# sunshanlu/ORB_SLAM2_ROS2

Measured on AMD Instinct MI355X. Metric: stereo frames/sec (extract+match) KITTI-00 1241x376; HBM GB/s vs roofline, higher is better.
Workload: dtype u8; 1 GPU; Single 1241x376 KITTI-shaped stereo pair, 8-level pyramid, 2000 FAST+rBRIEF keypoints per image, searchByStereo; batched (512 pairs per step, 512 of them distinct synthetic frames).  `value` is DEVICE-RESIDENT; the checks, rooflines, host_io, sequence job, content sweep, CPU baseline and extra legs run with --full; io=device-resident, n_features=2000, levels=8

## Files before the change

### include/orbfe.h

```cpp
#ifndef ORBFE_H_
#define ORBFE_H_

#include <stddef.h>
#include <stdint.h>

#ifdef __cplusplus
extern "C" {
#endif

#define ORBFE_ABI_VERSION 4
#define ORBFE_MAX_LEVELS 16
#define ORBFE_DESC_BYTES 32

typedef enum orbfe_status {
  ORBFE_OK = 0,
  ORBFE_EBADARG = 1,
  ORBFE_EBADSIZE = 2,
  ORBFE_EDEVICE = 3,
  ORBFE_ECAPACITY = 4,
  ORBFE_ENOMEM = 5
} orbfe_status;

typedef struct orbfe_keypoint {
  float x, y;
// ... 427 lines not shown
orbfe_status orbfe_kfstore_erase(orbfe_kfstore* store, int32_t n, const uint64_t* ids);
orbfe_status orbfe_kfstore_size(orbfe_kfstore* store, int64_t* n_keyframes, int64_t* bytes_used, int64_t* bytes_reserved);
orbfe_status orbfe_kfstore_info_get(orbfe_kfstore* store, uint64_t id, orbfe_kfstore_info* out);
orbfe_status orbfe_kfstore_fetch(orbfe_kfstore* store, uint64_t id, orbfe_keypoint* kps, uint8_t* desc, double* depth, double* right_u,
                                 int32_t* cell_off, int32_t* cell_feat, uint32_t* nodes, int32_t* node_offsets, uint32_t* features);
orbfe_status orbfe_fuse_into_keyframes_stored(orbfe_ctx* ctx, orbfe_kfstore* store, uint64_t cur_id, int32_t n_cur, const orbfe_fuse_points* pts,
                                              int32_t n_kf, const uint64_t* target_ids, const orbfe_fuse_pose* poses ,
                                              const float* z , const orbfe_camera* cam, float bl, const float* scale_factors,
                                              int32_t n_levels, float th, float ratio, int32_t dist_threshold, int32_t* best_idx,
                                              int32_t* best_dist, uint8_t* visible);
orbfe_status orbfe_create_new_map_points_stored(orbfe_ctx* ctx, orbfe_kfstore* store, uint64_t cur_id, const orbfe_tri_state* cur, int32_t n_nb,
                                                const uint64_t* nb_ids, const orbfe_tri_state* nbs, const orbfe_camera* cam, const float* k_inv,
                                                float bl, const float* scale_factors, int32_t n_levels, orbfe_tri_record* records, int64_t cap,
                                                int64_t* n_records, int32_t* tail, int64_t tail_cap, int64_t* n_tail, uint8_t* consumed);

typedef enum orbfe_stage {
  ORBFE_STAGE_RESIZE = 0,
  ORBFE_STAGE_BLUR = 1,
  ORBFE_STAGE_FAST = 2,
  ORBFE_STAGE_QUADTREE = 3,
  ORBFE_STAGE_BRIEF = 4,
  ORBFE_STAGE_STEREO = 5,
  ORBFE_STAGE_MATCH = 6,
  ORBFE_STAGE_BA = 7,
  ORBFE_STAGE_COUNT = 8
} orbfe_stage;
orbfe_status orbfe_profile_enable(orbfe_ctx* ctx, int32_t on);
orbfe_status orbfe_profile_read(orbfe_ctx* ctx, double* ms , int64_t* launches , int32_t reset);
const char* orbfe_stage_name(int32_t stage);

orbfe_status orbfe_debug_candidates(orbfe_ctx* ctx, int32_t slot, int32_t level, float* xyr, int32_t cap, int32_t* n_out);
orbfe_status orbfe_debug_se3_oplus(orbfe_ctx* ctx, int32_t n, const double* poses , const double* upd ,
                                   double* out );

#ifdef __cplusplus
}
#endif
#endif
```

### orb_slam2_ros2_amd/_lib.py

```python
from __future__ import annotations

import ctypes as C
import threading
import os

import numpy as np

_HERE = os.path.dirname(os.path.abspath(__file__))
LIB_PATH = os.path.join(_HERE, "liborbfe_hip.so")

KP_DTYPE = np.dtype(
    [("x", "<f4"), ("y", "<f4"), ("size", "<f4"), ("angle", "<f4"), ("response", "<f4"), ("octave", "<i4"), ("class_id", "<i4")]
)
assert KP_DTYPE.itemsize == 28

ORBFE_OK = 0
STATUS_NAMES = {0: "OK", 1: "EBADARG", 2: "EBADSIZE", 3: "EDEVICE", 4: "ECAPACITY", 5: "ENOMEM"}
STAGE_COUNT = 8


class OrbfeError(RuntimeError):
    def __init__(self, status: int, msg: str):
        super().__init__(f"orbfe {STATUS_NAMES.get(status, status)}: {msg}")
        self.status = status
# ... 119 lines not shown


class TriState(C.Structure):
    _fields_ = [("n", C.c_int32), ("flags", C.c_void_p), ("Tcw", C.c_float * 16), ("Twc", C.c_float * 16), ("Ow", C.c_float * 3),
                ("unproc", C.c_void_p), ("unproc_pos", C.c_void_p)]


FUSE_MAX_KF = 64
TRI_REC_DTYPE = np.dtype([("nb", "<i4"), ("q", "<i4"), ("t", "<i4"), ("kind", "<i4"), ("xyz", "<f4", (3,))])
TRI_MAX_NB = 64


class BaEdgeOut(C.Structure):
    _fields_ = [("error", C.c_void_p), ("chi2", C.c_void_p), ("rho", C.c_void_p), ("j_point", C.c_void_p),
                ("j_pose", C.c_void_p), ("depth_positive", C.c_void_p)]


EXPORTS = [
    "orbfe_abi_version", "orbfe_create", "orbfe_destroy", "orbfe_last_error", "orbfe_get_level_info", "orbfe_get_scale_factors",
    "orbfe_get_capacity",
    "orbfe_extract", "orbfe_extract_batch", "orbfe_extract_slot", "orbfe_extract_slot_begin", "orbfe_extract_slot_end", "orbfe_extract_slots", "orbfe_frame_stereo", "orbfe_frame_stereo_slots", "orbfe_frame_rgbd_image", "orbfe_track_motion_model", "orbfe_fetch_batch", "orbfe_fetch_stereo_batch", "orbfe_get_pyramid", "orbfe_stereo_match", "orbfe_stereo_batch_device", "orbfe_sync",
    "orbfe_host_alloc", "orbfe_host_alloc_on", "orbfe_host_free", "orbfe_recommended_hw_queues", "orbfe_stream_submit", "orbfe_stream_wait", "orbfe_stream_device_results", "orbfe_record_bytes", "orbfe_stream_pack_records",
    "orbfe_fetch_features", "orbfe_fetch_stereo", "orbfe_device_results", "orbfe_match_bruteforce", "orbfe_ba_eval_edges", "orbfe_ba_build_system", "orbfe_ba_local_optimize", "orbfe_pose_only_optimize", "orbfe_search_in_area", "orbfe_search_in_area_features", "orbfe_search_in_area_features_ex", "orbfe_extract_color", "orbfe_frame_rgbd", "orbfe_project_map_points", "orbfe_track_local_map",
    "orbfe_map_pb_summary", "orbfe_map_pb_reencode", "orbfe_map_pb_to_txt", "orbfe_map_txt_to_pb", "orbfe_map_local_graph", "orbfe_map_local_ba",
    "orbfe_vocab_load_txt", "orbfe_vocab_info_get", "orbfe_vocab_export", "orbfe_vocab_destroy", "orbfe_bow_transform", "orbfe_bow_slots",
    "orbfe_kfdb_create", "orbfe_kfdb_destroy", "orbfe_kfdb_add", "orbfe_kfdb_set_bad", "orbfe_kfdb_erase", "orbfe_kfdb_size", "orbfe_kfdb_query",
    "orbfe_kfdb_score", "orbfe_kfdb_group_filter",
    "orbfe_pnp_create", "orbfe_pnp_destroy", "orbfe_pnp_iterate", "orbfe_pnp_engine", "orbfe_pnp_stats",
    "orbfe_create_new_map_points", "orbfe_fuse_into_keyframes",
    "orbfe_kfstore_create", "orbfe_kfstore_destroy", "orbfe_kfstore_add", "orbfe_kfstore_add_from_slot", "orbfe_kfstore_set_bow",
    "orbfe_kfstore_erase", "orbfe_kfstore_size", "orbfe_kfstore_info_get", "orbfe_kfstore_fetch", "orbfe_fuse_into_keyframes_stored",
    "orbfe_create_new_map_points_stored",
    "orbfe_profile_enable", "orbfe_profile_read", "orbfe_stage_name", "orbfe_debug_candidates", "orbfe_debug_se3_oplus",
]
BOW_MAX_FEATURES = 65535

_lib = None


def load() -> C.CDLL:
    global _lib
    if _lib is not None:
        return _lib
    if not os.path.exists(LIB_PATH):
        raise OSError(f"{LIB_PATH} is missing: build it with `make -C orb_slam2_ros2_amd/csrc` "
                      "(there is no CPU fallback for the front end)")
    try:
        import torch
    except ImportError:
        pass
    L = C.CDLL(LIB_PATH)
    vp, i32, f32 = C.c_void_p, C.c_int32, C.c_float
    L.orbfe_abi_version.restype = C.c_int
    L.orbfe_create.argtypes = [C.POINTER(Config), C.POINTER(vp)]
    L.orbfe_destroy.argtypes = [vp]
    L.orbfe_destroy.restype = None
    L.orbfe_last_error.argtypes = [vp]
    L.orbfe_last_error.restype = C.c_char_p
    L.orbfe_get_level_info.argtypes = [vp, i32, C.POINTER(LevelInfo)]
    L.orbfe_get_scale_factors.argtypes = [vp, vp, i32]
    L.orbfe_get_capacity.argtypes = [vp]
    L.orbfe_get_capacity.restype = i32
    L.orbfe_extract.argtypes = [vp, vp, C.c_size_t, vp, vp, vp]
    L.orbfe_extract_batch.argtypes = [vp, i32, vp, C.c_size_t, vp, vp, vp]
    if hasattr(L, "orbfe_extract_slot_begin"):
        L.orbfe_extract_slot_begin.argtypes = [vp, i32, vp, C.c_size_t]
# ... 62 lines not shown
    L.orbfe_kfdb_score.argtypes = [vp, vp, C.POINTER(KfdbQueryIn), vp, i32, vp]
    L.orbfe_kfdb_group_filter.argtypes = [C.c_int64, vp, vp, vp, vp, vp, C.POINTER(C.c_int64)]
    L.orbfe_pnp_create.argtypes = [i32, i32, vp, vp, vp, vp, vp, i32, C.POINTER(Camera), C.POINTER(PnpParams), C.POINTER(vp)]
    L.orbfe_pnp_destroy.argtypes = [vp]
    L.orbfe_pnp_destroy.restype = None
    L.orbfe_pnp_iterate.argtypes = [vp, i32, i32, vp, C.POINTER(i32), vp, C.POINTER(C.c_int64), C.c_int64, C.POINTER(i32), C.POINTER(i32)]
    L.orbfe_pnp_engine.argtypes = [C.POINTER(C.c_uint32), C.POINTER(C.c_uint32)]
    L.orbfe_pnp_stats.argtypes = [vp, C.POINTER(C.c_int64), C.POINTER(C.c_int64)]
    L.orbfe_create_new_map_points.argtypes = [vp, C.POINTER(TriKf), i32, vp, C.POINTER(Camera), vp, f32, vp, i32, vp, C.c_int64,
                                              C.POINTER(C.c_int64), vp, C.c_int64, C.POINTER(C.c_int64), vp]
    L.orbfe_fuse_into_keyframes.argtypes = [vp, C.POINTER(FuseKf), C.POINTER(FusePoints), i32, vp, vp, C.POINTER(Camera), f32, vp, i32, f32, f32,
                                            i32, vp, vp, vp]
    u64, i64 = C.c_uint64, C.c_int64
    L.orbfe_kfstore_create.argtypes = [i32, i32, i32, i32, i64, C.POINTER(vp)]
    L.orbfe_kfstore_destroy.argtypes = [vp]
    L.orbfe_kfstore_destroy.restype = None
    L.orbfe_kfstore_add.argtypes = [vp, u64, i32, vp, vp, vp, vp, vp]
    L.orbfe_kfstore_add_from_slot.argtypes = [vp, vp, u64, i32, i32, vp, C.POINTER(i32)]
    L.orbfe_kfstore_set_bow.argtypes = [vp, u64, i32, vp, vp, vp]
    L.orbfe_kfstore_erase.argtypes = [vp, i32, vp]
    L.orbfe_kfstore_size.argtypes = [vp, C.POINTER(i64), C.POINTER(i64), C.POINTER(i64)]
    L.orbfe_kfstore_info_get.argtypes = [vp, u64, C.POINTER(KfstoreInfo)]
    L.orbfe_kfstore_fetch.argtypes = [vp, u64] + [vp] * 9
    L.orbfe_fuse_into_keyframes_stored.argtypes = [vp, vp, u64, i32, C.POINTER(FusePoints), i32, vp, vp, vp, C.POINTER(Camera), f32, vp, i32, f32,
                                                   f32, i32, vp, vp, vp]
    L.orbfe_create_new_map_points_stored.argtypes = [vp, vp, u64, C.POINTER(TriState), i32, vp, vp, C.POINTER(Camera), vp, f32, vp, i32, vp, i64,
                                                     C.POINTER(i64), vp, i64, C.POINTER(i64), vp]
    L.orbfe_profile_enable.argtypes = [vp, i32]
    L.orbfe_profile_read.argtypes = [vp, vp, vp, i32]
    L.orbfe_stage_name.argtypes = [i32]
    L.orbfe_stage_name.restype = C.c_char_p
    L.orbfe_debug_candidates.argtypes = [vp, i32, i32, vp, i32, vp]
    L.orbfe_debug_se3_oplus.argtypes = [vp, i32, vp, vp, vp]
    _lib = L
    return L


def ptr(a):
    return None if a is None else a.ctypes.data_as(C.c_void_p)


class PinnedArray:

    def __init__(self, shape, dtype, device_id=-1):
        self.lib = load()
        self.dtype = np.dtype(dtype)
        n = int(np.prod(shape)) * self.dtype.itemsize
        self.p = self.lib.orbfe_host_alloc_on(int(device_id), max(n, 1))
        if not self.p:
            raise MemoryError(f"orbfe_host_alloc({n}) failed")
        self.array = np.frombuffer((C.c_uint8 * max(n, 1)).from_address(self.p), dtype=self.dtype, count=int(np.prod(shape))).reshape(shape)

    def free(self):
        if getattr(self, "p", None):
            self.array = None
            self.lib.orbfe_host_free(self.p)
            self.p = None

    def __del__(self):
        try:
            self.free()
        except Exception:
            pass


def _status(st, what):
# ... 507 lines not shown
        self._check(self.lib.orbfe_fetch_batch(self.h, slot0, n_slots, ptr(kps), ptr(desc), ptr(cnt)))
        return kps, desc, cnt

    def fetch_stereo_batch(self, pair0, n_pairs):
        nf = max(self.n_features, 1)
        ru = np.zeros((n_pairs, nf), np.float64)
        dp = np.zeros((n_pairs, nf), np.float64)
        nm = np.zeros(n_pairs, np.int32)
        self._check(self.lib.orbfe_fetch_stereo_batch(self.h, pair0, n_pairs, ptr(ru), ptr(dp), ptr(nm)))
        return ru, dp, nm

    def pyramid(self, slot, level, blurred=False) -> np.ndarray:
        li = self.level_info(level)
        out = np.zeros((li.height, li.width), np.uint8)
        self._check(self.lib.orbfe_get_pyramid(self.h, slot, level, int(blurred), ptr(out)))
        return out

    def debug_candidates(self, slot, level) -> np.ndarray:
        n = C.c_int32(0)
        self._check(self.lib.orbfe_debug_candidates(self.h, slot, level, None, 0, C.byref(n)))
        out = np.zeros((max(n.value, 1), 3), np.float32)
        self._check(self.lib.orbfe_debug_candidates(self.h, slot, level, ptr(out), n.value, C.byref(n)))
        return out[:n.value]

    def debug_se3_oplus(self, poses, upd) -> np.ndarray:
        poses = np.ascontiguousarray(poses, np.float64).reshape(-1, 7)
        upd = np.ascontiguousarray(upd, np.float64).reshape(-1, 6)
        if poses.shape[0] != upd.shape[0]:
            raise ValueError("poses / upd disagree in length")
        n = poses.shape[0]
        out = np.zeros((max(n, 1), 7))
        self._check(self.lib.orbfe_debug_se3_oplus(self.h, n, ptr(poses), ptr(upd), ptr(out)))
        return out[:n]

    def stereo_match(self, slot_left, slot_right, fx, bf):
        nf = max(self.n_features, 1)
        ru = np.zeros(nf, np.float64)
        dp = np.zeros(nf, np.float64)
        br = np.zeros(nf, np.int32)
        bd = np.zeros(nf, np.int32)
        nm = C.c_int32(0)
        self._check(self.lib.orbfe_stereo_match(self.h, slot_left, slot_right, fx, bf, ptr(ru), ptr(dp), C.byref(nm), ptr(br), ptr(bd)))
        return nm.value, ru, dp, br, bd

    def stereo_batch_device(self, d_left_ptr, d_right_ptr, stride, image_pitch, n_pairs, fx, bf):
        self._check(self.lib.orbfe_stereo_batch_device(self.h, d_left_ptr, d_right_ptr, stride, image_pitch, n_pairs, fx, bf))

    def sync(self):
        self._check(self.lib.orbfe_sync(self.h))

    def alloc_batch_results(self, n_pairs, pinned=True):
        nf = max(self.n_features, 1)
        spec = dict(kps=((2 * n_pairs, nf), KP_DTYPE), desc=((2 * n_pairs, nf, 32), np.uint8), counts=((2 * n_pairs,), np.int32),
                    right_u=((n_pairs, nf), np.float64), depth=((n_pairs, nf), np.float64), n_matches=((n_pairs,), np.int32))
        out, keep = {}, []
        for k, (shape, dt) in spec.items():
            if pinned:
                pa = PinnedArray(shape, dt)
                keep.append(pa)
                out[k] = pa.array
            else:
                out[k] = np.zeros(shape, dt)
        out["_pinned"] = keep
        return out

    def stream_submit(self, left, right, n_pairs, fx, bf, out, stride=None, image_pitch=None):
# ... 523 lines not shown
```

### orb_slam2_ros2_amd/csrc/k_brief.hip

```cpp
#include <hip/hip_runtime.h>
#include <cstdio>
#include <cstring>

#include "orb_math.h"
#include "orbfe_internal.h"
#ifdef BRIEF_STAMPS
namespace orbfe { extern __device__ unsigned long long g_rt_t[4][8]; }
#define RT_STAMP(k) { __syncthreads(); if (tid == 0 && blockIdx.y == 0) orbfe::g_rt_t[k][0] = __builtin_amdgcn_s_memrealtime(); }
#define RTP_STAMP(k) { __syncthreads(); if (tid == 0 && blockIdx.y == 0) orbfe::g_rt_t[k][r] = __builtin_amdgcn_s_memrealtime(); }
#endif
#include "rowtable_body.h"
#include "wave_ops.h"

namespace orbfe {

typedef unsigned long long UmaxPacked;

template <int CTRL, int ROW_MASK>
__device__ __forceinline__ int dpp_i32(int v) {
  return __builtin_amdgcn_update_dpp(0, v, CTRL, ROW_MASK, 0xf, false);
}
__device__ __forceinline__ int wave_sum_i(int v) {
  v += dpp_i32<0x111, 0xf>(v);
  v += dpp_i32<0x112, 0xf>(v);
  v += dpp_i32<0x114, 0xf>(v);
  v += dpp_i32<0x118, 0xf>(v);
  v += dpp_i32<0x142, 0xa>(v);
  v += dpp_i32<0x143, 0xc>(v);
  return __builtin_amdgcn_readlane(v, 63);
}

__device__ __forceinline__ int locate_level(const int32_t* __restrict__ sc, int n_levels, int k, int* j_out, int* total_out) {
  int level = -1, acc = 0, j = 0;
  for (int l = 0; l < n_levels; ++l) {
    const int c = sc[l];
    if (level < 0 && k < acc + c) {
// ... 260 lines not shown

#ifndef BRIEF_WAVES
#define BRIEF_WAVES 4
#endif
#ifndef BRIEF_KPW
#define BRIEF_KPW 2
#endif
#ifdef BRIEF_STAMPS
__device__ unsigned long long g_rt_t[4][8];
__device__ unsigned long long g_bs_rec[8192][6];
#define BS_DECL const unsigned bs_w = ((blockIdx.y * 520u + blockIdx.x) * BRIEF_WAVES + (threadIdx.x >> 6)) & 8191u; const unsigned long long bs_t0 = __builtin_amdgcn_s_memrealtime(); unsigned long long bs_t1 = 0, bs_ta = 0, bs_tb = 0;
#define BS_MID if (!bs_t1) bs_t1 = __builtin_amdgcn_s_memrealtime();
#define BS_END(kind) if ((threadIdx.x & 63) == 0) { asm volatile("s_waitcnt vmcnt(0) lgkmcnt(0)" ::: "memory"); g_bs_rec[bs_w][0] = bs_t0, g_bs_rec[bs_w][1] = bs_t1, g_bs_rec[bs_w][2] = __builtin_amdgcn_s_memrealtime(), g_bs_rec[bs_w][3] = kind, g_bs_rec[bs_w][4] = bs_ta, g_bs_rec[bs_w][5] = bs_tb; }
#else
#define BS_DECL
#define BS_MID
#define BS_END(kind)
#endif
struct BriefRowTable {
  const KpAux* aux;
  const int32_t* n_kp;
  uint32_t* rowoff;
  uint16_t* rowlist;
  int32_t* n_match;
  int rows, list_cap, slot0, n_brief_blocks;
  int stage_cap;
  int32_t* flags;
};
__global__ __launch_bounds__(64 * BRIEF_WAVES) __attribute__((amdgpu_waves_per_eu(8, 8))) void k_brief(const uint8_t* __restrict__ blur, size_t img_pitch,
                                              const uint4* __restrict__ kpl, int n_features, const int8_t* __restrict__ pattern,
                                              const double2* __restrict__ sincos, uint8_t* __restrict__ desc, uint8_t* __restrict__ desc_host,
                                              BriefRowTable rt) {
#pragma clang fp contract(off)
  struct __attribute__((aligned(16))) Lds {
    double rc[BRIEF_WAVES][40];
    uint32_t win[BRIEF_WAVES][BRIEF_ROWS * BRIEF_WORDS + 1];
    double rs[BRIEF_WAVES][40];
  };
  static_assert(sizeof(double) * 40 * BRIEF_WAVES + sizeof(uint32_t) * (BRIEF_ROWS * BRIEF_WORDS + 1) * BRIEF_WAVES > 255 * 8 &&
                    (sizeof(double) * 40 * BRIEF_WAVES + sizeof(uint32_t) * (BRIEF_ROWS * BRIEF_WORDS + 1) * BRIEF_WAVES) % 512 != 0,
                "rc[w] and rs[w] must not be reachable by one ds_read2(st64)_b64");
  __shared__ Lds lds;
  BS_DECL
  if (rt.rowoff && (int)blockIdx.x >= rt.n_brief_blocks) {
    static_assert(sizeof(Lds) >= 9000, "the table's row counters borrow the descriptor kernel's LDS (launch_orient_brief checks the row count against 9000 bytes)");
    uint32_t* cnt = (uint32_t*)&lds;
    const int slot = rt.slot0 + (int)blockIdx.y;
    const int r = (int)blockIdx.x - rt.n_brief_blocks;
    if (rt.flags) {
      if (r == 0 && threadIdx.x == 0) rt.n_match[slot >> 1] = 0;
      const int rpw = (rt.rows + 7) >> 3;
      extern __shared__ __attribute__((aligned(16))) uint2 brief_bands[];
      rowtable_build_part(rt.aux + (size_t)blockIdx.y * n_features, min(rt.n_kp[blockIdx.y], n_features), rt.rows, rt.list_cap,
                          rt.rowoff + (size_t)slot * (rt.rows + 1), rt.rowlist + (size_t)slot * rt.list_cap, cnt, cnt + rpw + 12, (int)threadIdx.x, r,
                          rt.flags + (size_t)blockIdx.y * 8, rt.stage_cap > 0 ? brief_bands : nullptr, rt.stage_cap / 4);
      BS_END(2)
      return;
    }
    if (r != 0) return;
    if (threadIdx.x == 0) rt.n_match[slot >> 1] = 0;
    extern __shared__ __attribute__((aligned(16))) uint16_t brief_stage[];
    rowtable_build(rt.aux + (size_t)blockIdx.y * n_features, min(rt.n_kp[blockIdx.y], n_features), rt.rows, rt.list_cap,
                   rt.rowoff + (size_t)slot * (rt.rows + 1), rt.rowlist + (size_t)slot * rt.list_cap, cnt, cnt + rt.rows, (int)threadIdx.x,
                   rt.stage_cap > 0 ? brief_stage : nullptr, rt.stage_cap);
    BS_END(2)
    return;
  }
  const int lane = threadIdx.x & 63;
  uint32_t* win = lds.win[threadIdx.x >> 6];
  double* rc = lds.rc[threadIdx.x >> 6];
  double* rs = lds.rs[threadIdx.x >> 6];
  const int per_xcd = rt.n_brief_blocks >> 3;
  const int kb = ((int)blockIdx.x & 7) * per_xcd + ((int)blockIdx.x >> 3);
  const int k0 = (kb * BRIEF_WAVES + (threadIdx.x >> 6)) * BRIEF_KPW;
  const int img = blockIdx.y;
  if (k0 >= n_features) return;
  const uint4* list = kpl + (size_t)img * n_features;
  const double2* sc = sincos + (size_t)img * n_features;
  const uint8_t* W = blur + (size_t)img * img_pitch;
  const int k_last = min(k0 + BRIEF_KPW, n_features) - 1;
  const uint32_t tp0 = *(const uint32_t*)(pattern + (0 * 64 + lane) * 4), tp1 = *(const uint32_t*)(pattern + (1 * 64 + lane) * 4);
  const uint32_t tp2 = *(const uint32_t*)(pattern + (2 * 64 + lane) * 4), tp3 = *(const uint32_t*)(pattern + (3 * 64 + lane) * 4);
#ifdef BRIEF_STAMPS
  asm volatile("s_waitcnt vmcnt(0)" :: "v"(tp0), "v"(tp1), "v"(tp2), "v"(tp3) : "memory");
  bs_t1 = __builtin_amdgcn_s_memrealtime();
#endif
  constexpr int NIT = (BRIEF_ROWS + 4) / 5;
  const int ll = min(lane, 54);
  const int r0 = (ll * 373) >> 12, c0 = ll - r0 * BRIEF_WORDS;
  const int r_last = min(r0 + 5 * (NIT - 1), BRIEF_ROWS - 1);
  static_assert(NIT == 8, "Stage holds eight window words");
  struct Stage {
    uint4 wa, wb;
    double2 scv;
  };
  auto request = [&](const uint4 e, int k, Stage& st) __attribute__((always_inline)) {
    const bool used = (e.x & 0xFFFFu) != 0xFFFFu;
    const int x = used ? (int)(e.x & 0xFFFFu) : BRIEF_R, y = used ? (int)(e.x >> 16) : BRIEF_R;
    const uint32_t plane = used ? e.z : 0u;
    const int stride = used ? (int)e.w : 0;
    const int xa = (x - BRIEF_R) & ~3;
    const uint32_t step = 5u * (uint32_t)__builtin_amdgcn_readfirstlane(stride);
    const uint32_t a0 = plane + (uint32_t)mad24u(y - BRIEF_R + r0, stride, xa + 4 * c0);
#define BRIEF_WLD(it) (*(const uint32_t*)(W + (a0 + (uint32_t)(it) * step)))
    st.wa.x = BRIEF_WLD(0), st.wa.y = BRIEF_WLD(1), st.wa.z = BRIEF_WLD(2), st.wa.w = BRIEF_WLD(3);
    st.wb.x = BRIEF_WLD(4), st.wb.y = BRIEF_WLD(5), st.wb.z = BRIEF_WLD(6);
#undef BRIEF_WLD
    st.wb.w = *(const uint32_t*)(W + (plane + (uint32_t)mad24u(y - BRIEF_R + r_last, stride, xa + 4 * c0)));
    st.scv = sc[k];
  };
  uint4 e_cur = list[k0];
  uint4 e_nxt = list[min(k0 + 1, k_last)];
#ifdef BRIEF_STAMPS
  asm volatile("s_waitcnt vmcnt(0)" ::: "memory");
  bs_ta = __builtin_amdgcn_s_memrealtime();
#endif
  Stage st_cur;
  request(e_cur, k0, st_cur);
#ifdef BRIEF_STAMPS
  asm volatile("s_waitcnt vmcnt(0)" ::: "memory");
  bs_tb = __builtin_amdgcn_s_memrealtime();
#endif
#pragma unroll
  for (int i = 0; i < BRIEF_KPW; ++i) {
    const int k = k0 + i;
    if (k > k_last) break;
    const uint4 e_nn = list[min(k + 2, k_last)];
    Stage st_nxt;
    if (i + 1 < BRIEF_KPW) request(e_nxt, min(k + 1, k_last), st_nxt);
    if ((e_cur.x & 0xFFFFu) != 0xFFFFu) {
      const int x = (int)(e_cur.x & 0xFFFFu), y = (int)(e_cur.x >> 16);
      const int xa = (x - BRIEF_R) & ~3;
      if (lane < 55) {
        win[lane] = st_cur.wa.x, win[lane + 55] = st_cur.wa.y, win[lane + 110] = st_cur.wa.z, win[lane + 165] = st_cur.wa.w;
        win[lane + 220] = st_cur.wb.x, win[lane + 275] = st_cur.wb.y, win[lane + 330] = st_cur.wb.z;
        if (r0 + 5 * (NIT - 1) < BRIEF_ROWS) win[lane + 385] = st_cur.wb.w;
      }
      const double sn = st_cur.scv.x, cs = st_cur.scv.y;
      if (lane <= 2 * BRIEF_R) {
        const double v = (double)(float)(lane - BRIEF_R);
        rc[lane] = v * cs;
        rs[lane] = v * sn;
      }
      __builtin_amdgcn_fence(__ATOMIC_RELEASE, "wavefront");
      __builtin_amdgcn_wave_barrier();
      BS_MID
      const float px = (float)x, py = (float)y;
      typedef const __attribute__((address_space(3))) uint8_t* lds_bytes_t;
      const int y0w = y - BRIEF_R;
      const float magic_y = (float)(12582912 - (y0w & ~1));
      const float magic_x = (float)(12582912 - xa + (int)(uint32_t)(uintptr_t)(lds_bytes_t)(const uint8_t*)win - (y0w & 1) * (BRIEF_WORDS * 4));
      auto tests = [&](const uint32_t tpg) __attribute__((always_inline)) -> unsigned long long {
        const int x1 = (int)(int8_t)(tpg & 255u), y1 = (int)(int8_t)((tpg >> 8) & 255u);
        const int x2 = (int)(int8_t)((tpg >> 16) & 255u), y2 = (int)(int8_t)(tpg >> 24);
        const float p1x = (float)(rc[x1 + BRIEF_R] - rs[y1 + BRIEF_R]);
        const float p1y = (float)(rs[x1 + BRIEF_R] + rc[y1 + BRIEF_R]);
        const float p2x = (float)(rc[x2 + BRIEF_R] - rs[y2 + BRIEF_R]);
        const float p2y = (float)(rs[x2 + BRIEF_R] + rc[y2 + BRIEF_R]);
        const uint32_t a1 = (uint32_t)mad24u(__float_as_int((py + p1y) + magic_y), BRIEF_WORDS * 4, __float_as_int((px + p1x) + magic_x)) & 0xFFFFu;
        const uint32_t a2 = (uint32_t)mad24u(__float_as_int((py + p2y) + magic_y), BRIEF_WORDS * 4, __float_as_int((px + p2x) + magic_x)) & 0xFFFFu;
        const int v1 = *(lds_bytes_t)(uintptr_t)a1;
        const int v2 = *(lds_bytes_t)(uintptr_t)a2;
        return __ballot(v1 < v2);
      };
      const unsigned long long bits0 = tests(tp0), bits1 = tests(tp1), bits2 = tests(tp2), bits3 = tests(tp3);
      if (lane < 4) {
        unsigned long long* d64 = (unsigned long long*)(desc + ((size_t)img * n_features + k) * 32);
        unsigned long long b = bits0;
        if (lane == 1) b = bits1;
        if (lane == 2) b = bits2;
        if (lane == 3) b = bits3;
        d64[lane] = b;
        if (desc_host) ((unsigned long long*)(desc_host + ((size_t)img * n_features + k) * 32))[lane] = b;
      }
      __builtin_amdgcn_fence(__ATOMIC_RELEASE, "wavefront");
      __builtin_amdgcn_wave_barrier();
    }
    if (i + 1 < BRIEF_KPW) {
      e_cur = e_nxt;
      e_nxt = e_nn;
      st_cur = st_nxt;
    }
  }
  BS_END(1)
}
#ifdef BRIEF_STAMPS
}
extern "C" void orbfe_debug_brief_stamps() {
  static unsigned long long rec[8192][6];
  (void)hipDeviceSynchronize();
  (void)hipMemcpyFromSymbol(rec, HIP_SYMBOL(orbfe::g_bs_rec), sizeof(rec));
  unsigned long long first = ~0ull, last = 0, n = 0, sum = 0, mx = 0, mid = 0, rt0 = 0, rt1 = 0, dlast = 0, sa = 0, sb = 0, ma = 0, mb = 0, smax = 0;
  for (int w = 0; w < 8192; ++w) {
    if (!rec[w][3]) continue;
    first = first < rec[w][0] ? first : rec[w][0], last = last > rec[w][2] ? last : rec[w][2];
    if (rec[w][3] == 1) {
      ++n, sum += rec[w][2] - rec[w][0], mx = mx > rec[w][2] - rec[w][0] ? mx : rec[w][2] - rec[w][0], mid += rec[w][1] ? rec[w][1] - rec[w][0] : 0;
      dlast = dlast > rec[w][2] ? dlast : rec[w][2];
      sa += rec[w][4] - rec[w][0], sb += rec[w][5] - rec[w][4];
      ma = ma > rec[w][4] - rec[w][0] ? ma : rec[w][4] - rec[w][0], mb = mb > rec[w][5] - rec[w][4] ? mb : rec[w][5] - rec[w][4];
    }
  }
  printf("BRIEF stamps (last launch): %llu descriptor waves, launch span %.2f us, last descriptor wave ends at %.2f us; wave mean %.2f max %.2f us, pattern words arrive after %.2f us (mean)\n",
         n, (last - first) * 0.01, (dlast - first) * 0.01, n ? sum * 0.01 / n : 0.0, mx * 0.01, n ? mid * 0.01 / n : 0.0);
  for (int w = 0; w < 8192; ++w)
    if (rec[w][3] == 1) smax = smax > rec[w][0] - first ? smax : rec[w][0] - first;
  printf("  pattern + list entries arrive after %.2f us (mean, max %.2f); window + sin/cos %.2f us later (mean, max %.2f); last descriptor wave starts at %.2f us\n",
         n ? sa * 0.01 / n : 0.0, ma * 0.01, n ? sb * 0.01 / n : 0.0, mb * 0.01, smax * 0.01);
  for (int w = 0; w < 8192; ++w)
    if (rec[w][3] == 2 && (w & 3) == 0) printf("  row-table workgroup: starts %.2f us, ends %.2f us after the launch's first wave\n", (rec[w][0] - first) * 0.01, (rec[w][2] - first) * 0.01);
  {
    unsigned long long rt[4][8];
    (void)hipMemcpyFromSymbol(rt, HIP_SYMBOL(orbfe::g_rt_t), sizeof(rt));
    for (int r = 0; r < 8; ++r)
      printf("  row table part %d (image 0): zeroed %.2f | counted %.2f | lower parts known %.2f | scattered %.2f us after the launch's first wave\n", r,
             (rt[0][r] - first) * 0.01, (rt[1][r] - first) * 0.01, (rt[2][r] - first) * 0.01, (rt[3][r] - first) * 0.01);
  }
  memset(rec, 0, sizeof(rec));
  (void)hipMemcpyToSymbol(HIP_SYMBOL(orbfe::g_bs_rec), rec, sizeof(rec));
  (void)rt0, (void)rt1;
}
namespace orbfe {
#endif

void launch_orient_brief(hipStream_t s, const LevelDev* d_lv, int n_levels, const uint8_t* d_pyr, const uint8_t* d_blur,
                         size_t img_pitch, const uint32_t* d_sel, const int32_t* d_sel_count, int n_features,
                         const int8_t* d_pattern, const int umax[16], orbfe_keypoint* d_kps, uint8_t* d_desc, KpAux* d_aux,
                         int32_t* d_n_kp, double* d_theta, int2* d_moments, double2* d_sincos, KpX* d_kx,
                         uint4* d_kpl, int rows0, int n_img, hipEvent_t before_brief, hipEvent_t before_lists, orbfe_keypoint* h_kps,
                         uint8_t* h_desc, int32_t* h_n_kp, bool fuse_small, uint32_t* d_rowoff_slot, uint16_t* d_rowlist_slot, int32_t* d_n_match,
                         int rt_rows, int rt_list_cap, int rt_slot0, int32_t* d_rt_flags) {
  if (n_img <= 0 || n_features <= 0) return;
  UmaxPacked u = 0;
  for (int i = 0; i < 16; ++i) u |= (unsigned long long)(umax[i] & 15) << (4 * i);
  if (fuse_small && n_img <= 2) {
    if (before_lists) (void)hipStreamWaitEvent(s, before_lists, 0);
    hipLaunchKernelGGL(k_list_moments_orient<true>, dim3((n_features + 15) / 16, n_img), dim3(256), 0, s, d_lv, n_levels, d_sel, d_sel_count, n_features,
                       d_pyr, img_pitch, u, d_kpl, d_moments, d_sincos, d_kps, d_aux, d_kx, d_theta, rows0, d_n_kp, h_kps, h_n_kp,
                       (d_rowoff_slot && d_rt_flags) ? d_rt_flags + (size_t)rt_slot0 * 8 : (int32_t*)nullptr);
    if (before_brief) (void)hipStreamWaitEvent(s, before_brief, 0);
    const int nb = (((n_features + BRIEF_WAVES * BRIEF_KPW - 1) / (BRIEF_WAVES * BRIEF_KPW)) + 7) & ~7;
    BriefRowTable rt{};
    rt.n_brief_blocks = nb;
    if (d_rowoff_slot && (size_t)(rt_rows + 4) * 4 <= 9000)
      rt = BriefRowTable{d_aux, d_n_kp, d_rowoff_slot, d_rowlist_slot, d_n_match, rt_rows, rt_list_cap, rt_slot0, nb, 0,
                         d_rt_flags ? d_rt_flags + (size_t)rt_slot0 * 8 : (int32_t*)nullptr};
    if (rt.rowoff && (rt.flags || rt_list_cap % 8 == 0)) rt.stage_cap = rt.flags ? 4 * std::min(n_features, 4096) : std::min(rt_list_cap, 20480);
    hipLaunchKernelGGL(k_brief, dim3(nb + (rt.rowoff ? 8 : 0), n_img), dim3(64 * BRIEF_WAVES), (size_t)rt.stage_cap * 2, s, d_blur, img_pitch, d_kpl, n_features,
                       d_pattern, d_sincos, d_desc, h_desc, rt);
#ifdef EXP_BRIEF_TWICE
    hipLaunchKernelGGL(k_brief, dim3(nb + (rt.rowoff ? 8 : 0), n_img), dim3(64 * BRIEF_WAVES), 0, s, d_blur, img_pitch, d_kpl, n_features, d_pattern,
                       d_sincos, d_desc, h_desc, rt);
#endif
    return;
  }
  hipLaunchKernelGGL(k_kplist, dim3((n_features + 255) / 256, n_img), dim3(256), 0, s, d_lv, n_levels, d_sel, d_sel_count, n_features,
// ... 15 lines not shown
```

### orb_slam2_ros2_amd/csrc/orbfe_api.hip

```cpp
#include "orbfe_ctx.h"

static const int8_t kEmbeddedPattern[256][4] = {
#include "brief_pattern.inc"
};

static thread_local std::string g_last_error;

orbfe_status fail(orbfe_ctx* c, orbfe_status st, const char* fmt, ...) {
  char buf[512];
  va_list ap;
  va_start(ap, fmt);
  vsnprintf(buf, sizeof buf, fmt, ap);
  va_end(ap);
  (void)c;
  g_last_error = buf;
  return st;
}


static void build_resize_axis(int s, int d, std::vector<ResizeTap>& out) {
  const double scale = 1.0 / ((double)d / s);
  for (int i = 0; i < d; ++i) {
    float f = (float)((i + 0.5) * scale - 0.5);
    int si = cv_floor_f(f);
// ... 927 lines not shown
    for (int s = 0; s < ns; ++s) {
      const int32_t k = cnt[(size_t)s];
      if (!k) continue;
      HIP_TRY(c, hipMemcpyAsync(rec.data() + n, c->d_scr_a + (size_t)slot * c->scratch_pitch + L.cand_base + (size_t)s * L.shard_cap, sizeof(uint32_t) * k,
                                hipMemcpyDeviceToHost, c->stream));
      n += k;
    }
    HIP_TRY(c, hipStreamSynchronize(c->stream));
    if (rec.empty()) rec.resize(1);
  } else {
    HIP_TRY(c, hipMemcpyAsync(&n, c->d_n_cand + (size_t)slot * c->cfg.n_levels + level, sizeof(int32_t), hipMemcpyDeviceToHost, c->stream));
    HIP_TRY(c, hipStreamSynchronize(c->stream));
    n = std::min<int32_t>(std::max(n, 0), (int32_t)L.cand_cap);
    rec.resize((size_t)std::max(n, 1));
    if (n) HIP_TRY(c, hipMemcpyAsync(rec.data(), c->d_scr_a + (size_t)slot * c->scratch_pitch + L.cand_base, sizeof(uint32_t) * n, hipMemcpyDeviceToHost, c->stream));
    HIP_TRY(c, hipStreamSynchronize(c->stream));
  }
  std::vector<std::pair<uint64_t, uint32_t>> keyed((size_t)n);
  for (int i = 0; i < n; ++i) {
    const uint32_t x = ORBFE_REC_X(rec[i]), y = ORBFE_REC_Y(rec[i]);
    const uint32_t jdx = std::min<uint32_t>((x - 3) / L.w_cell, L.n_cols - 1), idx = std::min<uint32_t>((y - 3) / L.h_cell, L.n_rows - 1);
    keyed[i] = {((uint64_t)(idx * L.n_cols + jdx) << 24) | ((uint64_t)y << 12) | x, rec[i]};
  }
  std::sort(keyed.begin(), keyed.end());
  for (int i = 0; i < n && xyr && i < cap; ++i) {
    xyr[3 * i] = (float)ORBFE_REC_X(keyed[i].second);
    xyr[3 * i + 1] = (float)ORBFE_REC_Y(keyed[i].second);
    xyr[3 * i + 2] = (float)ORBFE_REC_R(keyed[i].second);
  }
  *n_out = n;
  return ORBFE_OK;
}

}
```

### orb_slam2_ros2_amd/csrc/orbfe_ctx.h

```cpp
#pragma once
#include <hip/hip_runtime.h>
#include <sched.h>

#include <algorithm>
#include <cctype>
#include <cmath>
#include <cstdarg>
#include <cstdio>
#include <cstdlib>
#include <cstring>
#include <atomic>
#include <chrono>
#include <mutex>
#include <string>
#include <limits>
#include <memory>
#include <vector>

#include "orbfe_internal.h"
#include "scratch_layout.h"
#include "search_area_layout.h"

namespace orbfe {
void launch_resize(hipStream_t s, const LevelDev* d_lv, const RsTile* d_tiles, const int* n_tiles, const int* lds_bytes,
// ... 51 lines not shown
                      const double* bp, const double* Hll, const double* bl, const double* Hpl, const double* lambda_p, double* Dinv, double* W,
                      double* S, double* rhs, double* x, int* ok, double* poses, double* points, double* dxp, double* dxl, double* scale_out,
                      double* big_scratch);
size_t lm_big_bytes(int nf);
size_t lm_big_inv_bytes(int nf);
int lm_big_ld(int nf);
void launch_lm_big_init(hipStream_t s, const LmLaunch& L);
void launch_lba_classify(hipStream_t s, int n_edges, const double* chi2_last, const uint8_t* depth_pos, const uint8_t* is_stereo,
                         uint8_t* level, double* info_eff, double* delta_eff);
void launch_lba_final(hipStream_t s, int n_edges, const double* chi2, const uint8_t* depth_pos, const uint8_t* is_stereo, uint8_t* bad);
void launch_ba_edges(hipStream_t s, int n_edges, const double* d_poses, const double* d_points, const int32_t* d_edge_pose,
                     const int32_t* d_edge_point, const double* d_meas, const uint8_t* d_is_stereo, const double* d_info,
                     const double* d_delta, BaParamsDev prm, double* d_error, double* d_chi2, double* d_rho, double* d_jpoint,
                     double* d_jpose, uint8_t* d_depth_pos);
void launch_project_map_points(hipStream_t s, int n, const float* d_pos, const float* d_vdir, const float* d_max, const float* d_min,
                               const float* R, const float* t, const float* cam4, const float* bounds4, float log_sf, int max_level,
                               float* d_uv, float* d_dist, float* d_cos, int8_t* d_level, uint8_t* d_vis);
void launch_grid_build(hipStream_t s, const orbfe_keypoint* d_kps, const int32_t* d_n_kp, int n_cap, int rows, int cols, int32_t* d_cell_off,
                       int32_t* d_cell_feat);
void launch_search_area(hipStream_t s, const uint4* d_kpl, const uint8_t* d_desc, int width, int height, int rows, int cols,
                        const int32_t* d_cell_off, const int32_t* d_cell_feat, int nq, const float* d_qxy, const float* d_radius,
                        const int8_t* d_min_level, const int8_t* d_max_level, const uint8_t* d_q_desc, const uint8_t* d_exclude,
                        int32_t* d_best_idx, int32_t* d_best_dist, int32_t* d_second, int32_t* d_n_cand, int32_t* d_excluded_hits);
void launch_lm_build(hipStream_t s, const LmLaunch& L, int gate, int which, int write_last, bool with_poses);
void launch_lm_maxdiag(hipStream_t s, const LmLaunch& L, int gate);
void launch_lm_pairs(hipStream_t s, const LmLaunch& L);
void launch_lm_steps(hipStream_t s, const LmLaunch& L, int n);
void launch_lm_switch(hipStream_t s, const LmLaunch& L);
void launch_lm_final(hipStream_t s, const LmLaunch& L);
void launch_pose_only(hipStream_t s, int n, const double* Xw, const double* meas, const double* info, const float* sigma2,
                      const double* pose_in, BaParamsDev prm, double d_mono, double d_stereo, double* err, uint8_t* level,
                      uint8_t* robust, uint8_t* inlier, double* pose_out, int32_t* n_good, const int32_t* n_dev = nullptr);
void launch_debug_se3_oplus(hipStream_t s, int n, const double* poses, const double* upd, double* out);
void launch_track_queries(hipStream_t s, int n, const uint8_t* d_flags, const uint8_t* d_visible, const float* d_cos, const int8_t* d_level, float th,
                          const float* d_sigma2, int n_levels, float* d_radius, int8_t* d_min_level, int8_t* d_max_level);
void launch_track_claim(hipStream_t s, int n, const int32_t* d_n_cand, const int32_t* d_best_idx, const int32_t* d_best_dist, const int32_t* d_second,
                        int min_threshold, float ratio, int32_t* d_claim, int last_wins = 0, int32_t* d_n_accept = nullptr, uint8_t* d_accepted = nullptr);
void launch_track_edges(hipStream_t s, const orbfe_keypoint* d_kps, const int32_t* d_n_kp, int n_features, const int32_t* d_held, const int32_t* d_claim,
                        const uint8_t* d_mp_flags, const float* d_mp_pos, const double* d_right_u, const float* d_sigma2, const float* d_inv_sigma2,
                        int min_matches, int32_t* d_assigned, int32_t* d_edge_of, double* d_Xw, double* d_meas, double* d_info, float* d_sig,
                        int32_t* d_counts, int32_t unclaimed = 0x7F7F7F7F, const int32_t* d_n_accept = nullptr, int base_matches = 0);
}

using namespace orbfe;

static const int kGaussTaps[2][7] = {{18, 34, 48, 56, 48, 34, 18}, {18, 34, 49, 55, 49, 34, 18}};
static const int kMeanThreshold = 75;

struct orbfe_ctx {
  std::recursive_mutex api_mu;
  orbfe_config cfg;
  int device = 0;
  hipStream_t stream = nullptr;
  bool own_stream = false;
  struct GraphEntry {
    int slot0, n_img;
    bool want_kps, want_desc;
    bool stereo;
    float fx, bf;
    const uint8_t* stage;
    const uint8_t* pyr;
    hipGraphExec_t exec;
    bool rgbd = false;
    unsigned char rkey[72] = {0};
  };
  struct Lane {
// ... 289 lines not shown
```

Measured before the change: 110,700 stereo pairs/s.

## Rotate BRIEF tests in float with margin check and exact double fallback

Replaces the per-wave LDS tables of double-precision cos/sin products with direct single-precision rotation of each test point. A small margin check flags points whose rounded coordinate could differ from the exact double result, and only those are recomputed in double, with a wave-wide branch. Keypoint fields and rotation values are made wave-uniform with readfirstlane so they can live in scalar registers. The goal is to cut LDS traffic and double-precision work in the BRIEF kernel while keeping results bit-exact, at the cost of extra float ops and a divergent fallback path. A debug kernel and API are added so the exactness of the rotation can be checked.

```diff
diff --git a/include/orbfe.h b/include/orbfe.h
--- a/include/orbfe.h
+++ b/include/orbfe.h
@@ -483,6 +483,8 @@
 orbfe_status orbfe_debug_candidates(orbfe_ctx* ctx, int32_t slot, int32_t level, float* xyr, int32_t cap, int32_t* n_out);
 orbfe_status orbfe_debug_se3_oplus(orbfe_ctx* ctx, int32_t n, const double* poses , const double* upd ,
                                    double* out );
+orbfe_status orbfe_debug_brief_rotate(orbfe_ctx* ctx, int32_t n, const double* items , int32_t* xy_out ,
+                                      uint8_t* took_exact );
 
 #ifdef __cplusplus
 }
diff --git a/orb_slam2_ros2_amd/_lib.py b/orb_slam2_ros2_amd/_lib.py
--- a/orb_slam2_ros2_amd/_lib.py
+++ b/orb_slam2_ros2_amd/_lib.py
@@ -175,6 +175,7 @@
     "orbfe_kfstore_erase", "orbfe_kfstore_size", "orbfe_kfstore_info_get", "orbfe_kfstore_fetch", "orbfe_fuse_into_keyframes_stored",
     "orbfe_create_new_map_points_stored",
     "orbfe_profile_enable", "orbfe_profile_read", "orbfe_stage_name", "orbfe_debug_candidates", "orbfe_debug_se3_oplus",
+    "orbfe_debug_brief_rotate",
 ]
 BOW_MAX_FEATURES = 65535
 
@@ -303,6 +304,7 @@
     L.orbfe_stage_name.restype = C.c_char_p
     L.orbfe_debug_candidates.argtypes = [vp, i32, i32, vp, i32, vp]
     L.orbfe_debug_se3_oplus.argtypes = [vp, i32, vp, vp, vp]
+    L.orbfe_debug_brief_rotate.argtypes = [vp, i32, vp, vp, vp]
     _lib = L
     return L
 
@@ -876,6 +878,16 @@
         out = np.zeros((max(n, 1), 7))
         self._check(self.lib.orbfe_debug_se3_oplus(self.h, n, ptr(poses), ptr(upd), ptr(out)))
         return out[:n]
+
+    def debug_brief_rotate(self, items, chunk=4096):
+        items = np.ascontiguousarray(items, np.float64).reshape(-1, 4)
+        n = items.shape[0]
+        xy = np.zeros((n, 512, 2), np.int32)
+        flags = np.zeros((n, 512), np.uint8)
+        for a in range(0, n, chunk):
+            b = min(a + chunk, n)
+            self._check(self.lib.orbfe_debug_brief_rotate(self.h, b - a, ptr(items[a:b]), ptr(xy[a:b]), ptr(flags[a:b])))
+        return xy, flags
 
     def stereo_match(self, slot_left, slot_right, fx, bf):
         nf = max(self.n_features, 1)
diff --git a/orb_slam2_ros2_amd/csrc/brief_rotate.h b/orb_slam2_ros2_amd/csrc/brief_rotate.h
--- /dev/null
+++ b/orb_slam2_ros2_amd/csrc/brief_rotate.h
@@ -0,0 +1,85 @@
+#pragma once
+#include <math.h>
+#include <stdint.h>
+#include <string.h>
+
+#include "orb_math.h"
+
+#if defined(__HIP_DEVICE_COMPILE__)
+#define BRIEFROT_ANY_LANE(flag) (__ballot(flag) != 0ull)
+#define BRIEFROT_KEEP_IN_BRANCH(v) asm volatile("" : "+v"(v))
+#else
+#define BRIEFROT_ANY_LANE(flag) (flag)
+#define BRIEFROT_KEEP_IN_BRANCH(v) (void)(v)
+#endif
+
+namespace briefrot {
+
+constexpr float MAGIC = 12582912.0f;
+constexpr float MARGIN = 32.0f / 16777216.0f;
+constexpr int MAX_R2 = 338;
+
+struct Rot {
+  double c, s;
+  float cf, sf;
+};
+ORB_HD Rot make_rot(double c, double s) {
+  Rot r;
+  r.c = c, r.s = s, r.cf = (float)c, r.sf = (float)s;
+  return r;
+}
+
+ORB_HD uint32_t f2u(float v) {
+  uint32_t b;
+  memcpy(&b, &v, 4);
+  return b;
+}
+
+ORB_HD float round_sum(float pc, float p, float magic) {
+#if defined(__clang__)
+#pragma clang fp contract(off)
+#endif
+  const float sum = pc + p;
+  return sum + magic;
+}
+ORB_HD int32_t as_int(float a) { return (int32_t)(f2u(a) - 0x4B400000u); }
+
+ORB_HD void exact_point(float x, float y, const Rot& r, float px, float py, float mx, float my, float& ax, float& ay) {
+#if defined(__clang__)
+#pragma clang fp contract(off)
+#endif
+  const float qx = (float)((double)x * r.c - (double)y * r.s);
+  const float qy = (float)((double)x * r.s + (double)y * r.c);
+  ax = round_sum(px, qx, mx);
+  ay = round_sum(py, qy, my);
+}
+
+ORB_HD bool fast_point(float x, float y, const Rot& r, float px, float py, float mx, float my, float margin, float& ax, float& ay) {
+#if defined(__clang__)
+#pragma clang fp contract(off)
+#endif
+  const float ys = y * r.sf, yc = y * r.cf;
+  const float qx = fmaf(x, r.cf, -ys);
+  const float qy = fmaf(x, r.sf, yc);
+  const float xl = round_sum(px, qx - margin, mx), xh = round_sum(px, qx + margin, mx);
+  const float yl = round_sum(py, qy - margin, my), yh = round_sum(py, qy + margin, my);
+  ax = xl, ay = yl;
+  return ((f2u(xl) ^ f2u(xh)) | (f2u(yl) ^ f2u(yh))) == 0u;
+}
+
+ORB_HD unsigned rotate_test(float x1, float y1, float x2, float y2, const Rot& r, float px, float py, float mx, float my, float margin,
+                            float& a1x, float& a1y, float& a2x, float& a2y) {
+  const bool redo1 = !fast_point(x1, y1, r, px, py, mx, my, margin, a1x, a1y);
+  const bool redo2 = !fast_point(x2, y2, r, px, py, mx, my, margin, a2x, a2y);
+  if (BRIEFROT_ANY_LANE(redo1 || redo2)) {
+    BRIEFROT_KEEP_IN_BRANCH(x1);
+    BRIEFROT_KEEP_IN_BRANCH(y1);
+    BRIEFROT_KEEP_IN_BRANCH(x2);
+    BRIEFROT_KEEP_IN_BRANCH(y2);
+    if (redo1) exact_point(x1, y1, r, px, py, mx, my, a1x, a1y);
+    if (redo2) exact_point(x2, y2, r, px, py, mx, my, a2x, a2y);
+  }
+  return (redo1 ? 1u : 0u) | (redo2 ? 2u : 0u);
+}
+
+}
diff --git a/orb_slam2_ros2_amd/csrc/k_brief.hip b/orb_slam2_ros2_amd/csrc/k_brief.hip
--- a/orb_slam2_ros2_amd/csrc/k_brief.hip
+++ b/orb_slam2_ros2_amd/csrc/k_brief.hip
@@ -2,6 +2,7 @@
 #include <cstdio>
 #include <cstring>
 
+#include "brief_rotate.h"
 #include "orb_math.h"
 #include "orbfe_internal.h"
 #ifdef BRIEF_STAMPS
@@ -328,14 +329,10 @@
                                               const double2* __restrict__ sincos, uint8_t* __restrict__ desc, uint8_t* __restrict__ desc_host,
                                               BriefRowTable rt) {
 #pragma clang fp contract(off)
-  struct __attribute__((aligned(16))) Lds {
-    double rc[BRIEF_WAVES][40];
+  union __attribute__((aligned(16))) Lds {
     uint32_t win[BRIEF_WAVES][BRIEF_ROWS * BRIEF_WORDS + 1];
-    double rs[BRIEF_WAVES][40];
+    uint32_t rowtable[2250];
   };
-  static_assert(sizeof(double) * 40 * BRIEF_WAVES + sizeof(uint32_t) * (BRIEF_ROWS * BRIEF_WORDS + 1) * BRIEF_WAVES > 255 * 8 &&
-                    (sizeof(double) * 40 * BRIEF_WAVES + sizeof(uint32_t) * (BRIEF_ROWS * BRIEF_WORDS + 1) * BRIEF_WAVES) % 512 != 0,
-                "rc[w] and rs[w] must not be reachable by one ds_read2(st64)_b64");
   __shared__ Lds lds;
   BS_DECL
   if (rt.rowoff && (int)blockIdx.x >= rt.n_brief_blocks) {
@@ -364,8 +361,6 @@
   }
   const int lane = threadIdx.x & 63;
   uint32_t* win = lds.win[threadIdx.x >> 6];
-  double* rc = lds.rc[threadIdx.x >> 6];
-  double* rs = lds.rs[threadIdx.x >> 6];
   const int per_xcd = rt.n_brief_blocks >> 3;
   const int kb = ((int)blockIdx.x & 7) * per_xcd + ((int)blockIdx.x >> 3);
   const int k0 = (kb * BRIEF_WAVES + (threadIdx.x >> 6)) * BRIEF_KPW;
@@ -377,6 +372,14 @@
   const int k_last = min(k0 + BRIEF_KPW, n_features) - 1;
   const uint32_t tp0 = *(const uint32_t*)(pattern + (0 * 64 + lane) * 4), tp1 = *(const uint32_t*)(pattern + (1 * 64 + lane) * 4);
   const uint32_t tp2 = *(const uint32_t*)(pattern + (2 * 64 + lane) * 4), tp3 = *(const uint32_t*)(pattern + (3 * 64 + lane) * 4);
+  struct TestF {
+    float x1, y1, x2, y2;
+  };
+  auto unpack = [](const uint32_t tpg) __attribute__((always_inline)) -> TestF {
+    return TestF{(float)(int)(int8_t)(tpg & 255u), (float)(int)(int8_t)((tpg >> 8) & 255u), (float)(int)(int8_t)((tpg >> 16) & 255u),
+                 (float)(int)(int8_t)(tpg >> 24)};
+  };
+  const TestF tf0 = unpack(tp0), tf1 = unpack(tp1), tf2 = unpack(tp2), tf3 = unpack(tp3);
 #ifdef BRIEF_STAMPS
   asm volatile("s_waitcnt vmcnt(0)" :: "v"(tp0), "v"(tp1), "v"(tp2), "v"(tp3) : "memory");
   bs_t1 = __builtin_amdgcn_s_memrealtime();
@@ -405,7 +408,10 @@
     st.wb.w = *(const uint32_t*)(W + (plane + (uint32_t)mad24u(y - BRIEF_R + r_last, stride, xa + 4 * c0)));
     st.scv = sc[k];
   };
-  uint4 e_cur = list[k0];
+  auto uniform_u = [](uint32_t v) __attribute__((always_inline)) { return (uint32_t)__builtin_amdgcn_readfirstlane((int)v); };
+  auto uniform_f = [](float v) __attribute__((always_inline)) { return __int_as_float(__builtin_amdgcn_readfirstlane(__float_as_int(v))); };
+  auto uniform_e = [&](const uint4 e) __attribute__((always_inline)) { return make_uint4(uniform_u(e.x), uniform_u(e.y), uniform_u(e.z), uniform_u(e.w)); };
+  uint4 e_cur = uniform_e(list[k0]);
   uint4 e_nxt = list[min(k0 + 1, k_last)];
 #ifdef BRIEF_STAMPS
   asm volatile("s_waitcnt vmcnt(0)" ::: "memory");
@@ -432,48 +438,43 @@
         win[lane + 220] = st_cur.wb.x, win[lane + 275] = st_cur.wb.y, win[lane + 330] = st_cur.wb.z;
         if (r0 + 5 * (NIT - 1) < BRIEF_ROWS) win[lane + 385] = st_cur.wb.w;
       }
-      const double sn = st_cur.scv.x, cs = st_cur.scv.y;
-      if (lane <= 2 * BRIEF_R) {
-        const double v = (double)(float)(lane - BRIEF_R);
-        rc[lane] = v * cs;
-        rs[lane] = v * sn;
-      }
+      briefrot::Rot rot = briefrot::make_rot(st_cur.scv.y, st_cur.scv.x);
+      rot.cf = uniform_f(rot.cf), rot.sf = uniform_f(rot.sf);
       __builtin_amdgcn_fence(__ATOMIC_RELEASE, "wavefront");
       __builtin_amdgcn_wave_barrier();
       BS_MID
-      const float px = (float)x, py = (float)y;
+      const float px = uniform_f((float)x), py = uniform_f((float)y);
       typedef const __attribute__((address_space(3))) uint8_t* lds_bytes_t;
       const int y0w = y - BRIEF_R;
-      const float magic_y = (float)(12582912 - (y0w & ~1));
-      const float magic_x = (float)(12582912 - xa + (int)(uint32_t)(uintptr_t)(lds_bytes_t)(const uint8_t*)win - (y0w & 1) * (BRIEF_WORDS * 4));
-      auto tests = [&](const uint32_t tpg) __attribute__((always_inline)) -> unsigned long long {
-        const int x1 = (int)(int8_t)(tpg & 255u), y1 = (int)(int8_t)((tpg >> 8) & 255u);
-        const int x2 = (int)(int8_t)((tpg >> 16) & 255u), y2 = (int)(int8_t)(tpg >> 24);
-        const float p1x = (float)(rc[x1 + BRIEF_R] - rs[y1 + BRIEF_R]);
-        const float p1y = (float)(rs[x1 + BRIEF_R] + rc[y1 + BRIEF_R]);
-        const float p2x = (float)(rc[x2 + BRIEF_R] - rs[y2 + BRIEF_R]);
-        const float p2y = (float)(rs[x2 + BRIEF_R] + rc[y2 + BRIEF_R]);
-        const uint32_t a1 = (uint32_t)mad24u(__float_as_int((py + p1y) + magic_y), BRIEF_WORDS * 4, __float_as_int((px + p1x) + magic_x)) & 0xFFFFu;
-        const uint32_t a2 = (uint32_t)mad24u(__float_as_int((py + p2y) + magic_y), BRIEF_WORDS * 4, __float_as_int((px + p2x) + magic_x)) & 0xFFFFu;
+      const float magic_y = uniform_f((float)(12582912 - (y0w & ~1)));
+      const float magic_x = uniform_f((float)(12582912 - xa + (int)(uint32_t)(uintptr_t)(lds_bytes_t)(const uint8_t*)win - (y0w & 1) * (BRIEF_WORDS * 4)));
+      auto tests = [&](const TestF& t) __attribute__((always_inline)) -> unsigned long long {
+        float a1x, a1y, a2x, a2y;
+        briefrot::rotate_test(t.x1, t.y1, t.x2, t.y2, rot, px, py, magic_x, magic_y, briefrot::MARGIN, a1x, a1y, a2x, a2y);
+        const uint32_t a1 = (uint32_t)mad24u(__float_as_int(a1y), BRIEF_WORDS * 4, __float_as_int(a1x)) & 0xFFFFu;
+        const uint32_t a2 = (uint32_t)mad24u(__float_as_int(a2y), BRIEF_WORDS * 4, __float_as_int(a2x)) & 0xFFFFu;
         const int v1 = *(lds_bytes_t)(uintptr_t)a1;
         const int v2 = *(lds_bytes_t)(uintptr_t)a2;
         return __ballot(v1 < v2);
       };
-      const unsigned long long bits0 = tests(tp0), bits1 = tests(tp1), bits2 = tests(tp2), bits3 = tests(tp3);
+      const unsigned long long bits0 = tests(tf0), bits1 = tests(tf1), bits2 = tests(tf2), bits3 = tests(tf3);
       if (lane < 4) {
-        unsigned long long* d64 = (unsigned long long*)(desc + ((size_t)img * n_features + k) * 32);
+        const int ks = __builtin_amdgcn_readfirstlane(k);
+        uint32_t lane8 = (uint32_t)lane * 8u;
+        asm volatile("" : "+v"(lane8));
+        unsigned long long* d64 = (unsigned long long*)(desc + ((size_t)img * n_features + ks) * 32 + lane8);
         unsigned long long b = bits0;
         if (lane == 1) b = bits1;
         if (lane == 2) b = bits2;
         if (lane == 3) b = bits3;
-        d64[lane] = b;
-        if (desc_host) ((unsigned long long*)(desc_host + ((size_t)img * n_features + k) * 32))[lane] = b;
+        *d64 = b;
+        if (desc_host) *(unsigned long long*)(desc_host + ((size_t)img * n_features + ks) * 32 + lane8) = b;
       }
       __builtin_amdgcn_fence(__ATOMIC_RELEASE, "wavefront");
       __builtin_amdgcn_wave_barrier();
     }
     if (i + 1 < BRIEF_KPW) {
-      e_cur = e_nxt;
+      e_cur = uniform_e(e_nxt);
       e_nxt = e_nn;
       st_cur = st_nxt;
     }
@@ -518,6 +519,30 @@
 }
 namespace orbfe {
 #endif
+
+__global__ __launch_bounds__(64) void k_debug_brief_rotate(const double* __restrict__ items, const int8_t* __restrict__ pattern,
+                                                           int32_t* __restrict__ out, uint8_t* __restrict__ took_exact) {
+#pragma clang fp contract(off)
+  const size_t i = blockIdx.x;
+  const int lane = threadIdx.x;
+  const briefrot::Rot rot = briefrot::make_rot(items[i * 4], items[i * 4 + 1]);
+  const float px = (float)items[i * 4 + 2], py = (float)items[i * 4 + 3];
+  for (int g = 0; g < 4; ++g) {
+    const int j = g * 64 + lane;
+    const int8_t* t = pattern + j * 4;
+    float a1x, a1y, a2x, a2y;
+    const unsigned redo = briefrot::rotate_test((float)t[0], (float)t[1], (float)t[2], (float)t[3], rot, px, py, briefrot::MAGIC, briefrot::MAGIC,
+                                                briefrot::MARGIN, a1x, a1y, a2x, a2y);
+    int32_t* o = out + (i * 512 + 2 * (size_t)j) * 2;
+    o[0] = briefrot::as_int(a1x), o[1] = briefrot::as_int(a1y), o[2] = briefrot::as_int(a2x), o[3] = briefrot::as_int(a2y);
+    took_exact[i * 512 + 2 * (size_t)j] = (uint8_t)(redo & 1u);
+    took_exact[i * 512 + 2 * (size_t)j + 1] = (uint8_t)(redo >> 1);
+  }
+}
+
+void launch_debug_brief_rotate(hipStream_t s, int n, const double* items, const int8_t* d_pattern, int32_t* out, uint8_t* took_exact) {
+  if (n > 0) hipLaunchKernelGGL(k_debug_brief_rotate, dim3(n), dim3(64), 0, s, items, d_pattern, out, took_exact);
+}
 
 void launch_orient_brief(hipStream_t s, const LevelDev* d_lv, int n_levels, const uint8_t* d_pyr, const uint8_t* d_blur,
                          size_t img_pitch, const uint32_t* d_sel, const int32_t* d_sel_count, int n_features,
diff --git a/orb_slam2_ros2_amd/csrc/orbfe_api.hip b/orb_slam2_ros2_amd/csrc/orbfe_api.hip
--- a/orb_slam2_ros2_amd/csrc/orbfe_api.hip
+++ b/orb_slam2_ros2_amd/csrc/orbfe_api.hip
@@ -983,4 +983,33 @@
   return ORBFE_OK;
 }
 
-}
+orbfe_status orbfe_debug_brief_rotate(orbfe_ctx* c, int32_t n, const double* items, int32_t* xy_out, uint8_t* took_exact) {
+  ApiLock api_lk(c);
+  if (!c || n < 0 || !items || !xy_out || !took_exact) return fail(c, ORBFE_EBADARG, "debug_brief_rotate: bad argument");
+  if (n == 0) return ORBFE_OK;
+  for (size_t i = 0; i < (size_t)n; ++i) {
+    const double cs = items[i * 4], sn = items[i * 4 + 1], px = items[i * 4 + 2], py = items[i * 4 + 3];
+    const double lim = 1.0 + 1.0 / 1099511627776.0, far = 2097152.0 - 19.0;
+    if (!(std::fabs(cs) <= lim) || !(std::fabs(sn) <= lim) || !(std::fabs(px) < far) || !(std::fabs(py) < far) || px != std::floor(px) || py != std::floor(py))
+      return fail(c, ORBFE_EBADARG, "debug_brief_rotate: an item is outside |cos|, |sin| <= 1, integer |x|, |y| < 2^21 - 19");
+  }
+  HIP_TRY(c, hipSetDevice(c->device));
+  TRY(join_stereo(c));
+  const size_t N = (size_t)n;
+  ScratchLayout L;
+  ScratchRegion up, down;
+  const size_t o_i = L.open(up).take<double>(N * 4), o_x = L.close(up).open(down).take<int32_t>(N * 1024), o_f = L.take<uint8_t>(N * 512);
+  L.close(down);
+  StagedIo io;
+  TRY(io.reserve(c, L.end(), std::max(up.end, down.bytes())));
+  io.put(o_i, items, N * 32);
+  HIP_TRY(c, io.upload(up));
+  launch_debug_brief_rotate(c->stream, n, io.dev<double>(o_i), c->d_pattern, io.dev<int32_t>(o_x), io.dev<uint8_t>(o_f));
+  HIP_TRY(c, hipGetLastError());
+  HIP_TRY(c, io.fetch(down));
+  io.get(xy_out, o_x, N * 4096);
+  io.get(took_exact, o_f, N * 512);
+  return ORBFE_OK;
+}
+
+}
diff --git a/orb_slam2_ros2_amd/csrc/orbfe_ctx.h b/orb_slam2_ros2_amd/csrc/orbfe_ctx.h
--- a/orb_slam2_ros2_amd/csrc/orbfe_ctx.h
+++ b/orb_slam2_ros2_amd/csrc/orbfe_ctx.h
@@ -107,6 +107,7 @@
                       const double* pose_in, BaParamsDev prm, double d_mono, double d_stereo, double* err, uint8_t* level,
                       uint8_t* robust, uint8_t* inlier, double* pose_out, int32_t* n_good, const int32_t* n_dev = nullptr);
 void launch_debug_se3_oplus(hipStream_t s, int n, const double* poses, const double* upd, double* out);
+void launch_debug_brief_rotate(hipStream_t s, int n, const double* items, const int8_t* d_pattern, int32_t* out, uint8_t* took_exact);
 void launch_track_queries(hipStream_t s, int n, const uint8_t* d_flags, const uint8_t* d_visible, const float* d_cos, const int8_t* d_level, float th,
                           const float* d_sigma2, int n_levels, float* d_radius, int8_t* d_min_level, int8_t* d_max_level);
 void launch_track_claim(hipStream_t s, int n, const int32_t* d_n_cand, const int32_t* d_best_idx, const int32_t* d_best_dist, const int32_t* d_second,
```

Result: no change. 110,300 stereo pairs/s (-0.3%).
